# MiniMax-AI/VTP

Hardware: NVIDIA H100
Metric: images/sec (256x256 encode+decode+3-loss step) (higher is better)
Workload: dtype bf16

## Files before the change

vtp_b200/csrc/gemm.cu:

```cuda
#include <stdlib.h>

#include "host.h"
#include "ptx.cuh"

namespace vtp {

static constexpr int BM = 128;
static constexpr int BK = 64;
static constexpr int A_BYTES = BM * BK * 2;
static constexpr int NUM_THREADS = 512;
static constexpr int NUM_MMA_WARPS = 8;

struct GemmDev {
    int M, N, K;
    int a_mn, b_mn;
    int num_m_blocks, num_n_blocks, num_k_blocks, kb_per_split, num_splits;
    void* out;
    int ldo, out_dtype;
    const float* bias;
    int act, round_bf16;
    const void* resid;
    int ldr, resid_dtype;
    int accumulate;
    int rr_group, rr_skip;
    const __nv_bfloat16* rope_sin;
    const __nv_bfloat16* rope_cos;
    int rope_tokens, rope_prefix, rope_cols;
    int ps_r, ps_gh, ps_gw, ps_cout;
    __nv_bfloat16* out2;
    int ldo2;
    int conv_C, conv_H, conv_W, conv_TW, conv_TH, conv_tiles_h, conv_tiles_w, conv_B;
    const __nv_bfloat16* mask_pos;
    int ldm;
};

__device__ __forceinline__ float gelu_erf(float x) { return 0.5f * x * (1.0f + erff(x * 0.70710678118654752f)); }

static constexpr int STG_FLOATS = 32 * 32;
static constexpr int NUM_EPI_WARPS = 4;

__device__ __forceinline__ int stg_off(int r, int chunk ) { return r * 32 + ((chunk ^ (r & 7)) << 2); }

__device__ __forceinline__ long out_row(const GemmDev& p, int grow) {
    if (p.conv_C) {
// ... 246 lines not shown
            __syncwarp();
            store_bf16(p, stgb, lane, orow8, ocol0, 64, Nout, 0, has_resid);
            __syncwarp();
        }
        return;
    }
#pragma unroll
    for (int h = 0; h < 2; ++h) {
        if (32 * h < ncols) {
            stage_half(stg, lane, v, h);
            __syncwarp();
            store_half<PS>(p, stg, lane, grow0, orow8, ocol0, h, ncols, Nout, 0, has_resid);
            __syncwarp();
        }
    }
}


__device__ __forceinline__ int acc_key(int r) { return ((r & 3) << 1) | ((r >> 2) & 1); }

__device__ __forceinline__ void acc_ld32(const float* arow, int col0, int key, uint32_t (&r)[32]) {
#pragma unroll
    for (int i = 0; i < 8; ++i) {
        const float4 v = *reinterpret_cast<const float4*>(arow + col0 + 4 * (i ^ key));
        r[4 * i] = __float_as_uint(v.x), r[4 * i + 1] = __float_as_uint(v.y), r[4 * i + 2] = __float_as_uint(v.z),
        r[4 * i + 3] = __float_as_uint(v.w);
    }
}

struct AccHandoff {
    uint64_t* full;
    uint64_t* empty;
    uint32_t phase;
    __device__ __forceinline__ void wait_full() const { mbar_wait(full, phase); }
    __device__ __forceinline__ void release(int lane) const {
        __syncwarp();
        if (lane == 0) mbar_arrive(empty);
    }
};

struct TileIter {
    int n, m, ks;
    int dn, dm, dks;
    int nn, nm;
    __device__ __forceinline__ TileIter(int t0, int stride, int num_n, int num_m) : nn(num_n), nm(num_m) {
        n = t0 % num_n;
        const int r = t0 / num_n;
        m = r % num_m, ks = r / num_m;
        dn = stride % num_n;
        const int rs = stride / num_n;
        dm = rs % num_m, dks = rs / num_m;
    }
    __device__ __forceinline__ void next() {
        n += dn, m += dm, ks += dks;
        if (n >= nn) n -= nn, ++m;
        if (m >= nm) m -= nm, ++ks;
    }
};

template <int BN, int FAST>
__device__ __forceinline__ void fast_swiglu_tile(const GemmDev& p, const CUtensorMap* tmO, const CUtensorMap* tmO2, uint8_t* stg,
                                                 uint8_t* stg2, float* bias_s, int lane, int q, const AccHandoff& ah,
                                                 const float* arow, int key, int m_blk, int n0) {
    static_assert(BN == 128, "one packed chunk pair = one 64-column hidden line per tile row");
    constexpr bool PRE = FAST == 6;
    const int m0 = m_blk * BM;
    const int N = p.N;
// ... 153 lines not shown
                    if (ACT == VTP_ACT_RELU) {
#pragma unroll
                        for (int k = 0; k < 8; ++k) v[k] = fmaxf(v[k], 0.f);
                    }
                    uint4 w;
                    w.x = pack_bf16x2(v[0], v[1]), w.y = pack_bf16x2(v[2], v[3]);
                    w.z = pack_bf16x2(v[4], v[5]), w.w = pack_bf16x2(v[6], v[7]);
                    if (MASK) {
                        auto keep = [](uint32_t x, uint32_t mm) {
                            const uint32_t lo = ((mm & 0x7FFFu) != 0u && (mm & 0x8000u) == 0u) ? 0x0000FFFFu : 0u;
                            const uint32_t hi = ((mm & 0x7FFF0000u) != 0u && (mm & 0x80000000u) == 0u) ? 0xFFFF0000u : 0u;
                            return x & (lo | hi);
                        };
                        w.x = keep(w.x, rr[i].x), w.y = keep(w.y, rr[i].y), w.z = keep(w.z, rr[i].z), w.w = keep(w.w, rr[i].w);
                    } else if (RES) {
                        w.x = add_bf16x2(w.x, rr[i].x), w.y = add_bf16x2(w.y, rr[i].y), w.z = add_bf16x2(w.z, rr[i].z),
                        w.w = add_bf16x2(w.w, rr[i].w);
                    }
                    *reinterpret_cast<uint4*>(stg + stgb_off(lane, i)) = w;
                }
            }
            if (RES && !last) load_resid(col0 + CW);
            fence_proxy_async_smem();
            __syncwarp();
            if (lane == 0) {
                if (p.conv_C) tma_store_4d(tmO, stg, col0, ctx * p.conv_TW, cty * p.conv_TH + q * (32 / p.conv_TW), cb);
                else tma_store_2d(tmO, stg, col0, m0 + q * 32);
                bulk_commit();
            }
        }
    }
}

template <int BN, int STAGES, int TA, int TB>
__device__ __forceinline__ void gemm_mainloop(float (&acc)[BN / 2], uint8_t* ring, uint64_t* full_bar, uint64_t* empty_bar,
                                              int& s, uint32_t& ph, int nkb, int wg, int lane) {
    constexpr int STAGE_BYTES = A_BYTES + BN * BK * 2;
    int prev = -1;
    for (int kb = 0; kb < nkb; ++kb) {
        mbar_wait(&full_bar[s], ph);
        const uint32_t a_base = smem_u32(ring + s * STAGE_BYTES) + wg * 8192;
        const uint32_t b_base = smem_u32(ring + s * STAGE_BYTES + A_BYTES);
        wgmma_fence();
#pragma unroll
        for (int j = 0; j < BK / 16; ++j) {
            const uint64_t ad = TA ? wgmma_desc_sw128(a_base + j * 2048, 8192, 1024) : wgmma_desc_sw128(a_base + j * 32, 0, 1024);
            const uint64_t bd = TB ? wgmma_desc_sw128(b_base + j * 2048, 8192, 1024) : wgmma_desc_sw128(b_base + j * 32, 0, 1024);
            const uint32_t sc = (kb > 0 || j > 0) ? 1u : 0u;
            if constexpr (BN == 128) wgmma_m64n128_ss<TA, TB>(acc, ad, bd, sc);
            else wgmma_m64n64_ss<TA, TB>(acc, ad, bd, sc);
        }
        wgmma_commit();
        wgmma_wait<1>();
        fence_regs(acc);
        if (prev >= 0 && lane == 0) mbar_arrive(&empty_bar[prev]);
        prev = s;
        if (++s == STAGES) s = 0, ph ^= 1;
    }
    wgmma_wait<0>();
    fence_regs(acc);
    if (prev >= 0 && lane == 0) mbar_arrive(&empty_bar[prev]);
}

template <int BN, int STAGES, int ACT, bool PS, int FAST>
__global__ void __launch_bounds__(NUM_THREADS, 1)
gemm_kernel(const __grid_constant__ CUtensorMap tmA, const __grid_constant__ CUtensorMap tmB,
            const __grid_constant__ CUtensorMap tmO, const __grid_constant__ CUtensorMap tmO2, const GemmDev p) {
    static_assert(BN == 64 || BN == 128, "tile width");
    constexpr int B_BYTES = BN * BK * 2;
    constexpr int STAGE_BYTES = A_BYTES + B_BYTES;
    extern __shared__ __align__(1024) uint8_t smem_raw[];
    uint8_t* smem = reinterpret_cast<uint8_t*>((reinterpret_cast<uintptr_t>(smem_raw) + 1023) & ~uintptr_t(1023));
    constexpr int STG_BYTES = NUM_EPI_WARPS * STG_FLOATS * 4 * (FAST == 6 ? 2 : 1);
    uint8_t* ring = smem;
    float* acc_s = reinterpret_cast<float*>(ring + STAGES * STAGE_BYTES);
    float* stg_base = acc_s + BM * BN;
    float* bias_base = reinterpret_cast<float*>(reinterpret_cast<uint8_t*>(stg_base) + STG_BYTES);
    uint64_t* full_bar = reinterpret_cast<uint64_t*>(reinterpret_cast<uint8_t*>(bias_base) + (FAST ? NUM_EPI_WARPS * 256 : 0));
    uint64_t* empty_bar = full_bar + STAGES;
    uint64_t* acc_full = empty_bar + STAGES;
    uint64_t* acc_empty = acc_full + 1;

    const int warp = threadIdx.x >> 5;
    const int lane = threadIdx.x & 31;
    const int work_id = blockIdx.x;
    const int work_stride = gridDim.x;

    if (warp == 0 && lane == 0) {
        tma_prefetch_desc(&tmA);
        tma_prefetch_desc(&tmB);
        if (FAST) tma_prefetch_desc(&tmO);
        if (FAST == 6) tma_prefetch_desc(&tmO2);
        for (int s = 0; s < STAGES; ++s) mbar_init(&full_bar[s], 1), mbar_init(&empty_bar[s], NUM_MMA_WARPS);
        mbar_init(acc_full, NUM_MMA_WARPS);
        mbar_init(acc_empty, NUM_EPI_WARPS);
        fence_barrier_init();
    }
    __syncthreads();

    const int num_tiles = p.num_m_blocks * p.num_n_blocks * p.num_splits;
    if (warp < 4) {
        setmaxnreg_dec<40>();
        if (warp == 0 && lane == 0) {
            int s = 0;
            uint32_t ph = 0;
            TileIter ti(work_id, work_stride, p.num_n_blocks, p.num_m_blocks);
            for (int t = work_id; t < num_tiles; t += work_stride, ti.next()) {
                const int n_blk = ti.n, m_blk = ti.m, ks = ti.ks;
                const int kb0 = ks * p.kb_per_split;
                const int kb1 = min(kb0 + p.kb_per_split, p.num_k_blocks);
                const int m0 = m_blk * BM, n0 = n_blk * BN;
                int cv_x0 = 0, cv_y0 = 0, cv_b = 0, cv_c = 0, cv_dx = -1, cv_dy = -1;
                if (p.conv_C) {
                    cv_x0 = (m_blk % p.conv_tiles_w) * p.conv_TW;
                    cv_y0 = ((m_blk / p.conv_tiles_w) % p.conv_tiles_h) * p.conv_TH;
                    cv_b = m_blk / (p.conv_tiles_w * p.conv_tiles_h);
                    if (kb0 != 0) {
                        const int cpk = p.conv_C >> 6, tap = kb0 / cpk;
                        cv_c = (kb0 % cpk) << 6, cv_dx = tap % 3 - 1, cv_dy = tap / 3 - 1;
                    }
                }
                for (int kb = kb0; kb < kb1; ++kb) {
                    mbar_wait(&empty_bar[s], ph ^ 1);
                    uint8_t* sa = ring + s * STAGE_BYTES;
                    uint8_t* sb = sa + A_BYTES;
                    mbar_expect_tx(&full_bar[s], STAGE_BYTES);
                    const int k0 = kb * BK;
                    if (p.conv_C) {
                        tma_load_4d(sa, &tmA, &full_bar[s], cv_c, cv_x0 + cv_dx, cv_y0 + cv_dy, cv_b);
                        cv_c += 64;
                        if (cv_c == p.conv_C) {
                            cv_c = 0;
                            if (++cv_dx == 2) cv_dx = -1, ++cv_dy;
                        }
                    } else if (!p.a_mn) {
                        tma_load_2d(sa, &tmA, &full_bar[s], k0, m0);
                    } else {
                        tma_load_2d(sa, &tmA, &full_bar[s], m0, k0);
                        tma_load_2d(sa + 8192, &tmA, &full_bar[s], m0 + 64, k0);
                    }
                    if (!p.b_mn) {
                        tma_load_2d(sb, &tmB, &full_bar[s], k0, n0);
                    } else {
#pragma unroll
                        for (int i = 0; i < BN / 64; ++i) tma_load_2d(sb + i * 8192, &tmB, &full_bar[s], n0 + 64 * i, k0);
                    }
                    if (++s == STAGES) s = 0, ph ^= 1;
                }
            }
        }
    } else if (warp < 4 + NUM_MMA_WARPS) {
        setmaxnreg_inc<144>();
        const int wg = (warp >> 2) - 1;
        const int tw = threadIdx.x & 127;
        int s = 0;
        uint32_t ph = 0, acc_ph = 0;
        TileIter ti(work_id, work_stride, p.num_n_blocks, p.num_m_blocks);
        for (int t = work_id; t < num_tiles; t += work_stride, ti.next()) {
            const int kb0 = ti.ks * p.kb_per_split;
            const int nkb = min(kb0 + p.kb_per_split, p.num_k_blocks) - kb0;
            float acc[BN / 2];
            if (p.a_mn) {
                if (p.b_mn) gemm_mainloop<BN, STAGES, 1, 1>(acc, ring, full_bar, empty_bar, s, ph, nkb, wg, lane);
                else gemm_mainloop<BN, STAGES, 1, 0>(acc, ring, full_bar, empty_bar, s, ph, nkb, wg, lane);
            } else {
                if (p.b_mn) gemm_mainloop<BN, STAGES, 0, 1>(acc, ring, full_bar, empty_bar, s, ph, nkb, wg, lane);
                else gemm_mainloop<BN, STAGES, 0, 0>(acc, ring, full_bar, empty_bar, s, ph, nkb, wg, lane);
            }
            mbar_wait(acc_empty, acc_ph ^ 1);
            {
                const int r0 = 64 * wg + 16 * (tw >> 5) + ((tw & 31) >> 2), c0 = 2 * (tw & 3);
                const int key = acc_key(r0);
#pragma unroll
                for (int j = 0; j < BN / 8; ++j) {
                    const int off = 4 * ((2 * j + (c0 >> 2)) ^ key) + (c0 & 3);
                    *reinterpret_cast<float2*>(acc_s + r0 * BN + off) = make_float2(acc[4 * j], acc[4 * j + 1]);
                    *reinterpret_cast<float2*>(acc_s + (r0 + 8) * BN + off) = make_float2(acc[4 * j + 2], acc[4 * j + 3]);
                }
            }
            __syncwarp();
            if (lane == 0) mbar_arrive(acc_full);
            acc_ph ^= 1;
        }
    } else {
        setmaxnreg_inc<184>();
        const int q = warp & 3;
        float* stg = stg_base + q * STG_FLOATS;
        const bool has_resid = p.resid != nullptr;
        const float* arow = acc_s + (q * 32 + lane) * BN;
        const int key = acc_key(lane);
        AccHandoff ah{acc_full, acc_empty, 0};
        TileIter ti(work_id, work_stride, p.num_n_blocks, p.num_m_blocks);
        for (int t = work_id; t < num_tiles; t += work_stride, ti.next(), ah.phase ^= 1) {
            const int m_blk = ti.m, n0 = ti.n * BN;
            const int m0 = m_blk * BM;
            const int grow0 = m0 + q * 32;
            if constexpr (FAST == 6 || FAST == 7) {
                uint8_t* st1 = reinterpret_cast<uint8_t*>(stg);
                uint8_t* st2 = FAST == 6 ? reinterpret_cast<uint8_t*>(stg_base) + (NUM_EPI_WARPS + q) * STG_FLOATS * 4 : st1;
                fast_swiglu_tile<BN, FAST>(p, &tmO, &tmO2, st1, st2, bias_base + q * 64, lane, q, ah, arow, key, m_blk, n0);
                continue;
            }
            if constexpr (FAST != 0) {
                fast_epilogue_tile<BN, ACT, FAST>(p, &tmO, reinterpret_cast<uint8_t*>(stg), bias_base + q * 64, lane, q, ah,
                                                  arow, key, m_blk, n0);
                continue;
            }
            constexpr bool sw = ACT == VTP_ACT_SWIGLU8;
            long orow8[8];
#pragma unroll
            for (int it = 0; it < 8; ++it) orow8[it] = out_row(p, grow0 + 4 * it + (lane >> 3));
            uint32_t hold[16];
            ah.wait_full();
#pragma unroll 1
            for (int u = 0; u < BN / 64; ++u) {
                const int col0 = n0 + u * 64;
                if (col0 >= p.N) break;
                if (has_resid)
                    prefetch_resid_l2(p, lane, orow8, sw ? col0 >> 1 : col0, sw ? 32 : 64, sw ? p.N >> 1 : p.N);
                uint32_t r0[32], r1[32];
                acc_ld32(arow, u * 64, key, r0);
                acc_ld32(arow, u * 64 + 32, key, r1);
                if (u == BN / 64 - 1 || col0 + 64 >= p.N) ah.release(lane);
                float v[64];
#pragma unroll
                for (int i = 0; i < 32; ++i) v[i] = __uint_as_float(r0[i]), v[32 + i] = __uint_as_float(r1[i]);
                epilogue_unit<ACT, PS>(p, stg, lane, v, grow0, orow8, col0, has_resid, sw ? (u & 1) : 0, hold);
            }
        }
        if (FAST && lane == 0) bulk_wait0();
    }
}

template <int BN, int STAGES, int ACT, bool PS, int FAST = 0>
static int launch_gemm(const CUtensorMap& tmA, const CUtensorMap& tmB, const GemmDev& p, cudaStream_t stream,
                       const CUtensorMap* tmO = nullptr, const CUtensorMap* tmO2 = nullptr) {
    constexpr int smem_bytes = 1024 + STAGES * (A_BYTES + BN * BK * 2) + BM * BN * 4 +
                               NUM_EPI_WARPS * STG_FLOATS * 4 * (FAST == 6 ? 2 : 1) + (FAST ? NUM_EPI_WARPS * 256 : 0) +
                               (2 * STAGES + 2) * 8;
    static_assert(smem_bytes <= 232448, "shared memory budget (227 KB per block)");
    static bool configured = false;
    if (!configured) {
        VTP_CUDA(cudaFuncSetAttribute(gemm_kernel<BN, STAGES, ACT, PS, FAST>, cudaFuncAttributeMaxDynamicSharedMemorySize,
                                      smem_bytes));
        configured = true;
    }
    const int work = p.num_m_blocks * p.num_n_blocks * p.num_splits;
    const int grid = work < num_sms() ? work : num_sms();
    gemm_kernel<BN, STAGES, ACT, PS, FAST><<<grid, NUM_THREADS, smem_bytes, stream>>>(tmA, tmB, tmO ? *tmO : tmA,
                                                                                     tmO2 ? *tmO2 : tmA, p);
    VTP_LAUNCH_CHECK();
    return VTP_OK;
}

}

using namespace vtp;

extern "C" int vtp_gemm_bf16(const vtp_gemm_args* a, vtp_stream_t stream_) {
    cudaStream_t stream = reinterpret_cast<cudaStream_t>(stream_);
    VTP_CHECK_ARG(a != nullptr, "gemm: null args");
    VTP_CHECK_ARG(a->M > 0 && a->N > 0 && a->K > 0, "gemm: bad shape M=%d N=%d K=%d", a->M, a->N, a->K);
    VTP_CHECK_ARG(a->A && a->B && a->out, "gemm: null pointer");
    VTP_CHECK_ARG(a->lda % 8 == 0 && a->ldb % 8 == 0, "gemm: lda/ldb must be multiples of 8 (16B TMA strides)");
    VTP_CHECK_ARG((reinterpret_cast<uintptr_t>(a->A) & 15) == 0 && (reinterpret_cast<uintptr_t>(a->B) & 15) == 0,
                  "gemm: A/B must be 16B aligned");
    VTP_CHECK_ARG((reinterpret_cast<uintptr_t>(a->out) & 15) == 0, "gemm: out must be 16B aligned");
    VTP_CHECK_ARG(a->N % 8 == 0, "gemm: N must be a multiple of 8");
    VTP_CHECK_ARG(a->out_dtype == VTP_F32 || a->out_dtype == VTP_BF16, "gemm: bad out dtype");
    VTP_CHECK_ARG(a->ldo % (a->out_dtype == VTP_F32 ? 4 : 8) == 0 || a->ps_r > 0, "gemm: ldo alignment");
    int split_k = a->split_k < 1 ? 1 : a->split_k;
    const bool auto_split = a->split_k < 0 && a->accumulate && a->out_dtype == VTP_F32 && a->act == VTP_ACT_NONE && !a->bias;
    VTP_CHECK_ARG(split_k == 1 || (a->accumulate && a->out_dtype == VTP_F32 && a->act == VTP_ACT_NONE && !a->bias),
                  "gemm: split_k needs accumulate=1, fp32 out, no bias/activation");
    VTP_CHECK_ARG(!a->accumulate || a->out_dtype == VTP_F32, "gemm: accumulate needs fp32 out");
    if (a->act == VTP_ACT_ROPE)
        VTP_CHECK_ARG(a->rope_sin && a->rope_cos && a->rope_tokens > 0 && a->rope_cols % 64 == 0, "gemm: bad rope args");
    if (a->act == VTP_ACT_SWIGLU8) VTP_CHECK_ARG(a->N % 16 == 0, "gemm: swiglu needs N %% 16 == 0");
    if (a->ps_r > 0)
        VTP_CHECK_ARG(a->ps_r % 4 == 0 && a->M % (a->ps_gh * a->ps_gw) == 0 && a->N == a->ps_cout * a->ps_r * a->ps_r,
                      "gemm: bad pixel-shuffle args");
    if (a->resid) VTP_CHECK_ARG(a->ldr % (a->resid_dtype == VTP_F32 ? 4 : 8) == 0, "gemm: ldr alignment");
    if (a->out2) VTP_CHECK_ARG(a->ldo2 % 8 == 0, "gemm: ldo2 alignment");
// ... 23 lines not shown
        double best = -1.0;
        for (int sp = 1; sp <= 64 && sp * 8 <= (nkb > 8 ? nkb : 8); ++sp) {
            const int kps = ceil_div(nkb, sp);
            const int real = ceil_div(nkb, kps);
            const long work = (long)tiles * real;
            if (sp > 1 && work > 3L * grid) break;
            const double eff = (double)work / ((double)ceil_div((int)work, grid) * grid);
            if (eff > best + 0.02) best = eff, split_k = sp;
        }
    }

    GemmDev p;
    memset(&p, 0, sizeof(p));
    p.M = a->M, p.N = a->N, p.K = a->K;
    p.a_mn = a->a_mn_major ? 1 : 0, p.b_mn = a->b_mn_major ? 1 : 0;
    p.num_m_blocks = ceil_div(a->M, BM);
    p.num_n_blocks = ceil_div(a->N, BN);
    p.num_k_blocks = ceil_div(a->K, BK);
    p.kb_per_split = ceil_div(p.num_k_blocks, split_k);
    p.num_splits = ceil_div(p.num_k_blocks, p.kb_per_split);
    p.out = a->out, p.ldo = a->ldo, p.out_dtype = a->out_dtype;
    p.bias = a->bias, p.act = a->act, p.round_bf16 = a->round_bf16;
    p.resid = a->resid, p.ldr = a->ldr, p.resid_dtype = a->resid_dtype;
    p.accumulate = a->accumulate;
    p.rr_group = a->rr_group, p.rr_skip = a->rr_skip;
    p.rope_sin = reinterpret_cast<const __nv_bfloat16*>(a->rope_sin);
    p.rope_cos = reinterpret_cast<const __nv_bfloat16*>(a->rope_cos);
    p.rope_tokens = a->rope_tokens, p.rope_prefix = a->rope_prefix, p.rope_cols = a->rope_cols;
    p.ps_r = a->ps_r, p.ps_gh = a->ps_gh, p.ps_gw = a->ps_gw, p.ps_cout = a->ps_cout;
    p.out2 = reinterpret_cast<__nv_bfloat16*>(a->out2), p.ldo2 = a->ldo2;
    p.mask_pos = reinterpret_cast<const __nv_bfloat16*>(a->mask_pos), p.ldm = a->ldm;

    CUtensorMap tmA, tmB;
    if (conv) {
        const int W = a->conv_W, H = a->conv_H, Cc = a->conv_C, Bimg = a->M / (H * W);
        p.conv_C = Cc, p.conv_H = H, p.conv_W = W, p.conv_B = Bimg;
        p.conv_TW = (W % 16 == 0) ? 16 : (W % 8 == 0 ? 8 : 4);
        p.conv_TH = 128 / p.conv_TW;
        p.conv_tiles_w = W / p.conv_TW, p.conv_tiles_h = ceil_div(H, p.conv_TH);
        p.num_m_blocks = Bimg * p.conv_tiles_h * p.conv_tiles_w;
        p.M = p.num_m_blocks * 128;
        uint64_t dims[4] = {(uint64_t)Cc, (uint64_t)W, (uint64_t)H, (uint64_t)Bimg};
        uint64_t strides[3] = {(uint64_t)Cc * 2, (uint64_t)W * Cc * 2, (uint64_t)H * W * Cc * 2};
        uint32_t box[4] = {64, (uint32_t)p.conv_TW, (uint32_t)p.conv_TH, 1};
        int rc = make_tmap_bf16(&tmA, a->A, 4, dims, strides, box);
        if (rc) return rc;
    } else {
        uint64_t dims[2], strides[1] = {(uint64_t)a->lda * 2};
        uint32_t box[2];
        if (!p.a_mn) dims[0] = a->K, dims[1] = a->M, box[0] = 64, box[1] = 128;
        else dims[0] = a->M, dims[1] = a->K, box[0] = 64, box[1] = 64;
        int rc = make_tmap_bf16(&tmA, a->A, 2, dims, strides, box);
        if (rc) return rc;
    }
    {
        uint64_t dims[2], strides[1] = {(uint64_t)a->ldb * 2};
        uint32_t box[2];
        if (!p.b_mn) dims[0] = a->K, dims[1] = a->N, box[0] = 64, box[1] = (uint32_t)BN;
        else dims[0] = a->N, dims[1] = a->K, box[0] = 64, box[1] = 64;
        int rc = make_tmap_bf16(&tmB, a->B, 2, dims, strides, box);
        if (rc) return rc;
    }
    if (fast_swiglu) {
        CUtensorMap tmH, tmP;
        {
            uint64_t dims[2] = {(uint64_t)a->N / 2, (uint64_t)a->M}, strides[1] = {(uint64_t)a->ldo * 2};
            uint32_t box[2] = {64, 32};
            int rc = make_tmap(&tmH, a->out, VTP_BF16, 2, dims, strides, box);
            if (rc) return rc;
        }
        if (a->out2) {
            uint64_t dims[2] = {(uint64_t)a->N, (uint64_t)a->M}, strides[1] = {(uint64_t)a->ldo2 * 2};
            uint32_t box[2] = {64, 32};
            int rc = make_tmap(&tmP, a->out2, VTP_BF16, 2, dims, strides, box);
            if (rc) return rc;
            return launch_gemm<128, 4, VTP_ACT_SWIGLU8, false, 6>(tmA, tmB, p, stream, &tmH, &tmP);
        }
        return launch_gemm<128, 4, VTP_ACT_SWIGLU8, false, 7>(tmA, tmB, p, stream, &tmH);
    }
    if (fast) {
        CUtensorMap tmO;
        const int esz = a->out_dtype == VTP_F32 ? 4 : 2;
        int rc;
        if (conv) {
            uint64_t dims[4] = {(uint64_t)a->N, (uint64_t)p.conv_W, (uint64_t)p.conv_H, (uint64_t)p.conv_B};
            uint64_t strides[3] = {(uint64_t)a->ldo * 2, (uint64_t)p.conv_W * a->ldo * 2, (uint64_t)p.conv_H * p.conv_W * a->ldo * 2};
            uint32_t box[4] = {64, (uint32_t)p.conv_TW, (uint32_t)(32 / p.conv_TW), 1};
            rc = make_tmap(&tmO, a->out, VTP_BF16, 4, dims, strides, box);
        } else {
            uint64_t dims[2] = {(uint64_t)a->N, (uint64_t)a->M}, strides[1] = {(uint64_t)a->ldo * esz};
            uint32_t box[2] = {(uint32_t)(128 / esz), 32};
            rc = make_tmap(&tmO, a->out, a->out_dtype, 2, dims, strides, box);
        }
        if (rc) return rc;
        const int mode = a->mask_pos ? 5 : (a->out_dtype == VTP_F32 ? 3 : 1) + (a->resid ? 1 : 0);
#define VTP_FAST_CFG(ACT_, MODE_)                                                                                     \
    return BN == 64 ? launch_gemm<64, 4, ACT_, false, MODE_>(tmA, tmB, p, stream, &tmO)                              \
                    : launch_gemm<128, 4, ACT_, false, MODE_>(tmA, tmB, p, stream, &tmO)
        if (mode == 5) VTP_FAST_CFG(VTP_ACT_NONE, 5);
#define VTP_FAST_ACT(ACT_)                                 \
    do {                                                   \
        switch (mode) {                                    \
            case 1: VTP_FAST_CFG(ACT_, 1);                 \
            case 2: VTP_FAST_CFG(ACT_, 2);                 \
            case 3: VTP_FAST_CFG(ACT_, 3);                 \
            default: VTP_FAST_CFG(ACT_, 4);                \
        }                                                  \
    } while (0)
        if (a->act == VTP_ACT_RELU) VTP_FAST_ACT(VTP_ACT_RELU);
        VTP_FAST_ACT(VTP_ACT_NONE);
#undef VTP_FAST_ACT
#undef VTP_FAST_CFG
    }
#define VTP_LAUNCH(ACT_, PS_)                                                              \
    return BN == 64 ? launch_gemm<64, 4, ACT_, PS_>(tmA, tmB, p, stream)                  \
                    : launch_gemm<128, 4, ACT_, PS_>(tmA, tmB, p, stream)
    if (a->ps_r > 0) {
        VTP_CHECK_ARG(a->act == VTP_ACT_NONE, "gemm: pixel shuffle has no activation");
        VTP_LAUNCH(VTP_ACT_NONE, true);
    }
    switch (a->act) {
        case VTP_ACT_NONE: VTP_LAUNCH(VTP_ACT_NONE, false);
        case VTP_ACT_GELU: VTP_LAUNCH(VTP_ACT_GELU, false);
        case VTP_ACT_SWIGLU8: return launch_gemm<128, 4, VTP_ACT_SWIGLU8, false>(tmA, tmB, p, stream);
        case VTP_ACT_ROPE: VTP_LAUNCH(VTP_ACT_ROPE, false);
        case VTP_ACT_RELU: VTP_LAUNCH(VTP_ACT_RELU, false);
        default: VTP_FAIL(VTP_ERR_ARG, "gemm: unknown activation %d", a->act);
    }
#undef VTP_LAUNCH
}
```

vtp_b200/csrc/ptx.cuh:

```cuda
#pragma once
#include <cuda_runtime.h>
#include <cuda_bf16.h>
#include <cuda.h>
#include <stdint.h>

namespace vtp {

__device__ __forceinline__ uint32_t smem_u32(const void* p) {
    return static_cast<uint32_t>(__cvta_generic_to_shared(p));
}
__device__ __forceinline__ uint32_t lane_id() { return threadIdx.x & 31; }

__device__ __forceinline__ bool elect_one() {
    uint32_t pred;
    asm volatile(
        "{\n\t.reg .pred p;\n\t"
        "elect.sync _|p, 0xffffffff;\n\t"
        "selp.u32 %0, 1, 0, p;\n\t}\n"
        : "=r"(pred));
    return pred != 0;
}

__device__ __forceinline__ void mbar_init(uint64_t* bar, uint32_t count) {
    asm volatile("mbarrier.init.shared::cta.b64 [%0], %1;" ::"r"(smem_u32(bar)), "r"(count));
}
__device__ __forceinline__ void fence_barrier_init() {
    asm volatile("fence.mbarrier_init.release.cluster;" ::: "memory");
}
__device__ __forceinline__ void mbar_expect_tx(uint64_t* bar, uint32_t bytes) {
    asm volatile("mbarrier.arrive.expect_tx.shared::cta.b64 _, [%0], %1;" ::"r"(smem_u32(bar)), "r"(bytes)
                 : "memory");
}
__device__ __forceinline__ void mbar_arrive(uint64_t* bar) {
    asm volatile("mbarrier.arrive.shared::cta.b64 _, [%0];" ::"r"(smem_u32(bar)) : "memory");
}
__device__ __forceinline__ bool mbar_try_wait(uint64_t* bar, uint32_t parity) {
    uint32_t ok;
    asm volatile(
        "{\n\t.reg .pred p;\n\t"
        "mbarrier.try_wait.parity.shared::cta.b64 p, [%1], %2;\n\t"
        "selp.u32 %0, 1, 0, p;\n\t}\n"
        : "=r"(ok)
        : "r"(smem_u32(bar)), "r"(parity)
        : "memory");
    return ok != 0;
}
__device__ __forceinline__ void mbar_wait(uint64_t* bar, uint32_t parity) {
    while (!mbar_try_wait(bar, parity)) {
    }
}

__device__ __forceinline__ uint32_t cluster_ctarank() {
    uint32_t r;
    asm volatile("mov.u32 %0, %%cluster_ctarank;" : "=r"(r));
    return r;
}
__device__ __forceinline__ void cluster_sync() {
    asm volatile("barrier.cluster.arrive.release.aligned;\n\tbarrier.cluster.wait.acquire.aligned;" ::: "memory");
}
__device__ __forceinline__ uint32_t mapa_shared(uint32_t saddr, uint32_t rank) {
    uint32_t r;
    asm volatile("mapa.shared::cluster.u32 %0, %1, %2;" : "=r"(r) : "r"(saddr), "r"(rank));
    return r;
}
__device__ __forceinline__ float4 ld_shared_cluster_f4(uint32_t caddr) {
    float4 v;
    asm volatile("ld.shared::cluster.v4.f32 {%0, %1, %2, %3}, [%4];"
                 : "=f"(v.x), "=f"(v.y), "=f"(v.z), "=f"(v.w)
                 : "r"(caddr)
                 : "memory");
    return v;
}

__device__ __forceinline__ void fence_proxy_async_smem() {
    asm volatile("fence.proxy.async.shared::cta;" ::: "memory");
}

__device__ __forceinline__ void tma_prefetch_desc(const CUtensorMap* m) {
    asm volatile("prefetch.tensormap [%0];" ::"l"(reinterpret_cast<uint64_t>(m)) : "memory");
}
__device__ __forceinline__ void tma_load_2d(void* dst, const CUtensorMap* m, uint64_t* bar, int x, int y) {
    asm volatile(
// ... 133 lines not shown
```

Measured before the change: 700.5.

## Add ping-pong GEMM variant where two warpgroups alternate mainloop and epilogue

Adds a ping-pong kernel variant with 384 threads: one producer warpgroup plus two consumer warpgroups. Each consumer computes a full 128-row tile (two m64 wgmmas) and then runs that tile's epilogue itself, alternating tiles with the other consumer. Named barriers order mainloop turns and staging-buffer reuse. The goal is to overlap one tile's epilogue with the next tile's tensor-core work, replacing the separate epilogue warps. It is chosen when BN is 64 or there are at least 32 K-blocks per split. In exchange it needs 240 registers per consumer thread and adds more complex barrier phasing.

Result: no change. 703.2 (median of 6 runs) (+0.4%).

```diff
diff --git a/vtp_b200/csrc/gemm.cu b/vtp_b200/csrc/gemm.cu
--- a/vtp_b200/csrc/gemm.cu
+++ b/vtp_b200/csrc/gemm.cu
@@ -10,6 +10,7 @@
 static constexpr int A_BYTES = BM * BK * 2;
 static constexpr int NUM_THREADS = 512;
 static constexpr int NUM_MMA_WARPS = 8;
+static constexpr int PP_THREADS = 384;
 
 struct GemmDev {
     int M, N, K;
@@ -322,7 +323,16 @@
     uint64_t* full;
     uint64_t* empty;
     uint32_t phase;
-    __device__ __forceinline__ void wait_full() const { mbar_wait(full, phase); }
+    uint64_t* stg_free = nullptr;
+    int bar_id = 0;
+    __device__ __forceinline__ void wait_full() const {
+        if (bar_id) {
+            named_bar_sync(bar_id, 128);
+            mbar_wait(stg_free, phase);
+        } else {
+            mbar_wait(full, phase);
+        }
+    }
     __device__ __forceinline__ void release(int lane) const {
         __syncwarp();
         if (lane == 0) mbar_arrive(empty);
@@ -572,8 +582,50 @@
     if (prev >= 0 && lane == 0) mbar_arrive(&empty_bar[prev]);
 }
 
-template <int BN, int STAGES, int ACT, bool PS, int FAST>
-__global__ void __launch_bounds__(NUM_THREADS, 1)
+template <int BN, int STAGES, int TA, int TB>
+__device__ __forceinline__ void gemm_mainloop_pp(float (&acc0)[BN / 2], float (&acc1)[BN / 2], uint8_t* ring, uint64_t* full_bar,
+                                              uint64_t* empty_bar, int kpos, int nkb, int next_bar, int lane) {
+    constexpr int STAGE_BYTES = A_BYTES + BN * BK * 2;
+    int s = kpos % STAGES;
+    uint32_t ph = (kpos / STAGES) & 1;
+    int prev = -1;
+    for (int kb = 0; kb < nkb; ++kb) {
+        mbar_wait(&full_bar[s], ph);
+        const uint32_t a_base = smem_u32(ring + s * STAGE_BYTES);
+        const uint32_t b_base = smem_u32(ring + s * STAGE_BYTES + A_BYTES);
+        wgmma_fence();
+#pragma unroll
+        for (int j = 0; j < BK / 16; ++j) {
+            const uint64_t ad0 = TA ? wgmma_desc_sw128(a_base + j * 2048, 8192, 1024) : wgmma_desc_sw128(a_base + j * 32, 0, 1024);
+            const uint64_t ad1 = TA ? wgmma_desc_sw128(a_base + 8192 + j * 2048, 8192, 1024)
+                                    : wgmma_desc_sw128(a_base + 8192 + j * 32, 0, 1024);
+            const uint64_t bd = TB ? wgmma_desc_sw128(b_base + j * 2048, 8192, 1024) : wgmma_desc_sw128(b_base + j * 32, 0, 1024);
+            const uint32_t sc = (kb > 0 || j > 0) ? 1u : 0u;
+            if constexpr (BN == 128) {
+                wgmma_m64n128_ss<TA, TB>(acc0, ad0, bd, sc);
+                wgmma_m64n128_ss<TA, TB>(acc1, ad1, bd, sc);
+            } else {
+                wgmma_m64n64_ss<TA, TB>(acc0, ad0, bd, sc);
+                wgmma_m64n64_ss<TA, TB>(acc1, ad1, bd, sc);
+            }
+        }
+        wgmma_commit();
+        if (kb == nkb - 1 && next_bar) named_bar_arrive(next_bar, 256);
+        wgmma_wait<1>();
+        fence_regs(acc0);
+        fence_regs(acc1);
+        if (prev >= 0 && lane == 0) mbar_arrive(&empty_bar[prev]);
+        prev = s;
+        if (++s == STAGES) s = 0, ph ^= 1;
+    }
+    wgmma_wait<0>();
+    fence_regs(acc0);
+    fence_regs(acc1);
+    if (prev >= 0 && lane == 0) mbar_arrive(&empty_bar[prev]);
+}
+
+template <int BN, int STAGES, int ACT, bool PS, int FAST, bool PP>
+__global__ void __launch_bounds__(PP ? PP_THREADS : NUM_THREADS, 1)
 gemm_kernel(const __grid_constant__ CUtensorMap tmA, const __grid_constant__ CUtensorMap tmB,
             const __grid_constant__ CUtensorMap tmO, const __grid_constant__ CUtensorMap tmO2, const GemmDev p) {
     static_assert(BN == 64 || BN == 128, "tile width");
@@ -601,8 +653,8 @@
         tma_prefetch_desc(&tmB);
         if (FAST) tma_prefetch_desc(&tmO);
         if (FAST == 6) tma_prefetch_desc(&tmO2);
-        for (int s = 0; s < STAGES; ++s) mbar_init(&full_bar[s], 1), mbar_init(&empty_bar[s], NUM_MMA_WARPS);
-        mbar_init(acc_full, NUM_MMA_WARPS);
+        for (int s = 0; s < STAGES; ++s) mbar_init(&full_bar[s], 1), mbar_init(&empty_bar[s], PP ? 4 : NUM_MMA_WARPS);
+        mbar_init(acc_full, PP ? 4 : NUM_MMA_WARPS);
         mbar_init(acc_empty, NUM_EPI_WARPS);
         fence_barrier_init();
     }
@@ -610,7 +662,8 @@
 
     const int num_tiles = p.num_m_blocks * p.num_n_blocks * p.num_splits;
     if (warp < 4) {
-        setmaxnreg_dec<40>();
+        if constexpr (PP) setmaxnreg_dec<24>();
+        else setmaxnreg_dec<40>();
         if (warp == 0 && lane == 0) {
             int s = 0;
             uint32_t ph = 0;
@@ -659,6 +712,92 @@
                 }
             }
         }
+    } else if constexpr (PP) {
+        uint64_t* const acc_free = acc_empty;
+        uint64_t* const stg_free = acc_full;
+        setmaxnreg_inc<240>();
+        const int wg = __shfl_sync(0xffffffffu, (warp >> 2) - 1, 0);
+        const int tw = threadIdx.x & 127;
+        const int q = warp & 3;
+        float* stg = stg_base + q * STG_FLOATS;
+        const bool has_resid = p.resid != nullptr;
+        const float* arow = acc_s + (q * 32 + lane) * BN;
+        const int key = acc_key(lane);
+        const AccHandoff ah{acc_full , acc_free, (uint32_t)(wg ^ 1), stg_free, 3 + wg};
+        const int my_turn = 1 + wg, other_turn = 2 - wg;
+        int kpos = 0;
+        TileIter ti(work_id, work_stride, p.num_n_blocks, p.num_m_blocks);
+        for (int t = work_id, j = 0; t < num_tiles; t += work_stride, ti.next(), ++j) {
+            const int kb0 = ti.ks * p.kb_per_split;
+            const int nkb = min(kb0 + p.kb_per_split, p.num_k_blocks) - kb0;
+            if ((j & 1) != wg) {
+                kpos += nkb;
+                continue;
+            }
+            const int next_bar = t + work_stride < num_tiles ? other_turn : 0;
+            if (j > 0) named_bar_sync(my_turn, 256);
+            float acc0[BN / 2], acc1[BN / 2];
+#pragma unroll
+            for (int i = 0; i < BN / 2; ++i) acc0[i] = 0.f, acc1[i] = 0.f;
+            if (p.a_mn) {
+                if (p.b_mn) gemm_mainloop_pp<BN, STAGES, 1, 1>(acc0, acc1, ring, full_bar, empty_bar, kpos, nkb, next_bar, lane);
+                else gemm_mainloop_pp<BN, STAGES, 1, 0>(acc0, acc1, ring, full_bar, empty_bar, kpos, nkb, next_bar, lane);
+            } else {
+                if (p.b_mn) gemm_mainloop_pp<BN, STAGES, 0, 1>(acc0, acc1, ring, full_bar, empty_bar, kpos, nkb, next_bar, lane);
+                else gemm_mainloop_pp<BN, STAGES, 0, 0>(acc0, acc1, ring, full_bar, empty_bar, kpos, nkb, next_bar, lane);
+            }
+            kpos += nkb;
+            mbar_wait(acc_free, ah.phase);
+            {
+                const int r0 = 16 * (tw >> 5) + ((tw & 31) >> 2), c0 = 2 * (tw & 3);
+                const int key0 = acc_key(r0);
+#pragma unroll
+                for (int jj = 0; jj < BN / 8; ++jj) {
+                    const int off = 4 * ((2 * jj + (c0 >> 2)) ^ key0) + (c0 & 3);
+                    *reinterpret_cast<float2*>(acc_s + r0 * BN + off) = make_float2(acc0[4 * jj], acc0[4 * jj + 1]);
+                    *reinterpret_cast<float2*>(acc_s + (r0 + 8) * BN + off) = make_float2(acc0[4 * jj + 2], acc0[4 * jj + 3]);
+                    *reinterpret_cast<float2*>(acc_s + (r0 + 64) * BN + off) = make_float2(acc1[4 * jj], acc1[4 * jj + 1]);
+                    *reinterpret_cast<float2*>(acc_s + (r0 + 72) * BN + off) = make_float2(acc1[4 * jj + 2], acc1[4 * jj + 3]);
+                }
+            }
+            const int m_blk = ti.m, n0 = ti.n * BN;
+            const int m0 = m_blk * BM;
+            const int grow0 = m0 + q * 32;
+            if constexpr (FAST == 6 || FAST == 7) {
+                uint8_t* st1 = reinterpret_cast<uint8_t*>(stg);
+                uint8_t* st2 = FAST == 6 ? reinterpret_cast<uint8_t*>(stg_base) + (NUM_EPI_WARPS + q) * STG_FLOATS * 4 : st1;
+                fast_swiglu_tile<BN, FAST>(p, &tmO, &tmO2, st1, st2, bias_base + q * 64, lane, q, ah, arow, key, m_blk, n0);
+            } else if constexpr (FAST != 0) {
+                fast_epilogue_tile<BN, ACT, FAST>(p, &tmO, reinterpret_cast<uint8_t*>(stg), bias_base + q * 64, lane, q, ah,
+                                                  arow, key, m_blk, n0);
+            } else {
+                constexpr bool sw = ACT == VTP_ACT_SWIGLU8;
+                long orow8[8];
+#pragma unroll
+                for (int it = 0; it < 8; ++it) orow8[it] = out_row(p, grow0 + 4 * it + (lane >> 3));
+                uint32_t hold[16];
+                ah.wait_full();
+#pragma unroll 1
+                for (int u = 0; u < BN / 64; ++u) {
+                    const int col0 = n0 + u * 64;
+                    if (col0 >= p.N) break;
+                    if (has_resid)
+                        prefetch_resid_l2(p, lane, orow8, sw ? col0 >> 1 : col0, sw ? 32 : 64, sw ? p.N >> 1 : p.N);
+                    uint32_t r0[32], r1[32];
+                    acc_ld32(arow, u * 64, key, r0);
+                    acc_ld32(arow, u * 64 + 32, key, r1);
+                    if (u == BN / 64 - 1 || col0 + 64 >= p.N) ah.release(lane);
+                    float v[64];
+#pragma unroll
+                    for (int i = 0; i < 32; ++i) v[i] = __uint_as_float(r0[i]), v[32 + i] = __uint_as_float(r1[i]);
+                    epilogue_unit<ACT, PS>(p, stg, lane, v, grow0, orow8, col0, has_resid, sw ? (u & 1) : 0, hold);
+                }
+            }
+            if (FAST && lane == 0) bulk_wait_read0();
+            __syncwarp();
+            if (lane == 0) mbar_arrive(stg_free);
+        }
+        if (FAST && lane == 0) bulk_wait0();
     } else if (warp < 4 + NUM_MMA_WARPS) {
         setmaxnreg_inc<144>();
         const int wg = (warp >> 2) - 1;
@@ -749,16 +888,21 @@
                                NUM_EPI_WARPS * STG_FLOATS * 4 * (FAST == 6 ? 2 : 1) + (FAST ? NUM_EPI_WARPS * 256 : 0) +
                                (2 * STAGES + 2) * 8;
     static_assert(smem_bytes <= 232448, "shared memory budget (227 KB per block)");
-    static bool configured = false;
-    if (!configured) {
-        VTP_CUDA(cudaFuncSetAttribute(gemm_kernel<BN, STAGES, ACT, PS, FAST>, cudaFuncAttributeMaxDynamicSharedMemorySize,
-                                      smem_bytes));
-        configured = true;
+    const bool pp = BN == 64 || p.kb_per_split >= 32;
+    static bool configured[2] = {false, false};
+    if (!configured[pp]) {
+        if (pp) VTP_CUDA(cudaFuncSetAttribute(gemm_kernel<BN, STAGES, ACT, PS, FAST, true>,
+                                              cudaFuncAttributeMaxDynamicSharedMemorySize, smem_bytes));
+        else VTP_CUDA(cudaFuncSetAttribute(gemm_kernel<BN, STAGES, ACT, PS, FAST, false>,
+                                           cudaFuncAttributeMaxDynamicSharedMemorySize, smem_bytes));
+        configured[pp] = true;
     }
     const int work = p.num_m_blocks * p.num_n_blocks * p.num_splits;
     const int grid = work < num_sms() ? work : num_sms();
-    gemm_kernel<BN, STAGES, ACT, PS, FAST><<<grid, NUM_THREADS, smem_bytes, stream>>>(tmA, tmB, tmO ? *tmO : tmA,
-                                                                                     tmO2 ? *tmO2 : tmA, p);
+    const CUtensorMap& o1 = tmO ? *tmO : tmA;
+    const CUtensorMap& o2 = tmO2 ? *tmO2 : tmA;
+    if (pp) gemm_kernel<BN, STAGES, ACT, PS, FAST, true><<<grid, PP_THREADS, smem_bytes, stream>>>(tmA, tmB, o1, o2, p);
+    else gemm_kernel<BN, STAGES, ACT, PS, FAST, false><<<grid, NUM_THREADS, smem_bytes, stream>>>(tmA, tmB, o1, o2, p);
     VTP_LAUNCH_CHECK();
     return VTP_OK;
 }
diff --git a/vtp_b200/csrc/ptx.cuh b/vtp_b200/csrc/ptx.cuh
--- a/vtp_b200/csrc/ptx.cuh
+++ b/vtp_b200/csrc/ptx.cuh
@@ -48,6 +48,13 @@
 __device__ __forceinline__ void mbar_wait(uint64_t* bar, uint32_t parity) {
     while (!mbar_try_wait(bar, parity)) {
     }
+}
+
+__device__ __forceinline__ void named_bar_sync(int id, int count) {
+    asm volatile("bar.sync %0, %1;" ::"r"(id), "r"(count) : "memory");
+}
+__device__ __forceinline__ void named_bar_arrive(int id, int count) {
+    asm volatile("bar.arrive %0, %1;" ::"r"(id), "r"(count) : "memory");
 }
 
 __device__ __forceinline__ uint32_t cluster_ctarank() {
```

## Load conv halo slabs once and reuse across three vertical taps

Applied to the files above, without the earlier changes.

For implicit-GEMM 3x3 convolutions, the producer now loads one taller A slab (tile height plus two halo rows) per channel block and x-offset. The MMA warps then reuse it for the three dy taps by offsetting the smem descriptor by a row of the tile, instead of issuing a separate A TMA load per tap. A second barrier ring manages slab lifetimes. The K iteration order changes to dy-innermost, which reindexes the B weight loads. Freed smem allows more B stages (8 or 5), and the path is restricted to split_k=1, non-transposed B, and none/relu activations. The aim is to cut A-side TMA traffic roughly threefold, at the cost of extra barrier logic and a dependency on the weight layout's tap ordering.

Result: no change. 703.8 before, 709.6 after (median of 6 runs) (+0.8%).

```diff
diff --git a/vtp_b200/csrc/gemm.cu b/vtp_b200/csrc/gemm.cu
--- a/vtp_b200/csrc/gemm.cu
+++ b/vtp_b200/csrc/gemm.cu
@@ -542,15 +542,31 @@
     }
 }
 
-template <int BN, int STAGES, int TA, int TB>
+__host__ __device__ constexpr int halo_slabs(int stages) { return 1 + (stages + 2) / 3; }
+static constexpr int HALO_STAGES_64 = 8, HALO_STAGES_128 = 5;
+static constexpr int HALO_SLAB_BYTES = (BM + 2 * 16) * BK * 2;
+
+struct HaloRing {
+    uint8_t* slabs;
+    uint64_t* full;
+    uint64_t* empty;
+    int sl;
+    uint32_t ph;
+};
+
+template <int BN, int STAGES, int TA, int TB, bool HALO>
 __device__ __forceinline__ void gemm_mainloop(float (&acc)[BN / 2], uint8_t* ring, uint64_t* full_bar, uint64_t* empty_bar,
-                                              int& s, uint32_t& ph, int nkb, int wg, int lane) {
-    constexpr int STAGE_BYTES = A_BYTES + BN * BK * 2;
+                                              int& s, uint32_t& ph, int nkb, int wg, int lane, HaloRing& hr, int tw_bytes) {
+    constexpr int A_STAGE = HALO ? 0 : A_BYTES;
+    constexpr int STAGE_BYTES = A_STAGE + BN * BK * 2;
     int prev = -1;
+    int dy = 0, prev_dy = 0, prev_sl = 0;
     for (int kb = 0; kb < nkb; ++kb) {
+        if (HALO && dy == 0) mbar_wait(&hr.full[hr.sl], hr.ph);
         mbar_wait(&full_bar[s], ph);
-        const uint32_t a_base = smem_u32(ring + s * STAGE_BYTES) + wg * 8192;
-        const uint32_t b_base = smem_u32(ring + s * STAGE_BYTES + A_BYTES);
+        const uint32_t a_base = HALO ? smem_u32(hr.slabs + hr.sl * HALO_SLAB_BYTES) + wg * 8192 + dy * tw_bytes
+                                     : smem_u32(ring + s * STAGE_BYTES) + wg * 8192;
+        const uint32_t b_base = smem_u32(ring + s * STAGE_BYTES + A_STAGE);
         wgmma_fence();
 #pragma unroll
         for (int j = 0; j < BK / 16; ++j) {
@@ -563,33 +579,51 @@
         wgmma_commit();
         wgmma_wait<1>();
         fence_regs(acc);
-        if (prev >= 0 && lane == 0) mbar_arrive(&empty_bar[prev]);
+        if (prev >= 0 && lane == 0) {
+            mbar_arrive(&empty_bar[prev]);
+            if (HALO && prev_dy == 2) mbar_arrive(&hr.empty[prev_sl]);
+        }
         prev = s;
         if (++s == STAGES) s = 0, ph ^= 1;
+        if constexpr (HALO) {
+            prev_dy = dy, prev_sl = hr.sl;
+            if (++dy == 3) {
+                dy = 0;
+                if (++hr.sl == halo_slabs(STAGES)) hr.sl = 0, hr.ph ^= 1;
+            }
+        }
     }
     wgmma_wait<0>();
     fence_regs(acc);
-    if (prev >= 0 && lane == 0) mbar_arrive(&empty_bar[prev]);
-}
-
-template <int BN, int STAGES, int ACT, bool PS, int FAST>
+    if (prev >= 0 && lane == 0) {
+        mbar_arrive(&empty_bar[prev]);
+        if (HALO && prev_dy == 2) mbar_arrive(&hr.empty[prev_sl]);
+    }
+}
+
+template <int BN, int STAGES, int ACT, bool PS, int FAST, bool HALO>
 __global__ void __launch_bounds__(NUM_THREADS, 1)
 gemm_kernel(const __grid_constant__ CUtensorMap tmA, const __grid_constant__ CUtensorMap tmB,
             const __grid_constant__ CUtensorMap tmO, const __grid_constant__ CUtensorMap tmO2, const GemmDev p) {
     static_assert(BN == 64 || BN == 128, "tile width");
     constexpr int B_BYTES = BN * BK * 2;
-    constexpr int STAGE_BYTES = A_BYTES + B_BYTES;
+    constexpr int STAGE_BYTES = (HALO ? 0 : A_BYTES) + B_BYTES;
+    constexpr int SLABS = halo_slabs(STAGES);
+    constexpr int SLAB_RING_BYTES = HALO ? SLABS * HALO_SLAB_BYTES : 0;
     extern __shared__ __align__(1024) uint8_t smem_raw[];
     uint8_t* smem = reinterpret_cast<uint8_t*>((reinterpret_cast<uintptr_t>(smem_raw) + 1023) & ~uintptr_t(1023));
     constexpr int STG_BYTES = NUM_EPI_WARPS * STG_FLOATS * 4 * (FAST == 6 ? 2 : 1);
     uint8_t* ring = smem;
-    float* acc_s = reinterpret_cast<float*>(ring + STAGES * STAGE_BYTES);
+    uint8_t* slabs = ring + STAGES * STAGE_BYTES;
+    float* acc_s = reinterpret_cast<float*>(slabs + SLAB_RING_BYTES);
     float* stg_base = acc_s + BM * BN;
     float* bias_base = reinterpret_cast<float*>(reinterpret_cast<uint8_t*>(stg_base) + STG_BYTES);
     uint64_t* full_bar = reinterpret_cast<uint64_t*>(reinterpret_cast<uint8_t*>(bias_base) + (FAST ? NUM_EPI_WARPS * 256 : 0));
     uint64_t* empty_bar = full_bar + STAGES;
     uint64_t* acc_full = empty_bar + STAGES;
     uint64_t* acc_empty = acc_full + 1;
+    uint64_t* slab_full = acc_empty + 1;
+    uint64_t* slab_empty = slab_full + SLABS;
 
     const int warp = threadIdx.x >> 5;
     const int lane = threadIdx.x & 31;
@@ -604,6 +638,8 @@
         for (int s = 0; s < STAGES; ++s) mbar_init(&full_bar[s], 1), mbar_init(&empty_bar[s], NUM_MMA_WARPS);
         mbar_init(acc_full, NUM_MMA_WARPS);
         mbar_init(acc_empty, NUM_EPI_WARPS);
+        if (HALO)
+            for (int s = 0; s < SLABS; ++s) mbar_init(&slab_full[s], 1), mbar_init(&slab_empty[s], NUM_MMA_WARPS);
         fence_barrier_init();
     }
     __syncthreads();
@@ -612,8 +648,8 @@
     if (warp < 4) {
         setmaxnreg_dec<40>();
         if (warp == 0 && lane == 0) {
-            int s = 0;
-            uint32_t ph = 0;
+            int s = 0, hsl = 0;
+            uint32_t ph = 0, hph = 0;
             TileIter ti(work_id, work_stride, p.num_n_blocks, p.num_m_blocks);
             for (int t = work_id; t < num_tiles; t += work_stride, ti.next()) {
                 const int n_blk = ti.n, m_blk = ti.m, ks = ti.ks;
@@ -630,32 +666,53 @@
                         cv_c = (kb0 % cpk) << 6, cv_dx = tap % 3 - 1, cv_dy = tap / 3 - 1;
                     }
                 }
-                for (int kb = kb0; kb < kb1; ++kb) {
-                    mbar_wait(&empty_bar[s], ph ^ 1);
-                    uint8_t* sa = ring + s * STAGE_BYTES;
-                    uint8_t* sb = sa + A_BYTES;
-                    mbar_expect_tx(&full_bar[s], STAGE_BYTES);
-                    const int k0 = kb * BK;
-                    if (p.conv_C) {
-                        tma_load_4d(sa, &tmA, &full_bar[s], cv_c, cv_x0 + cv_dx, cv_y0 + cv_dy, cv_b);
-                        cv_c += 64;
-                        if (cv_c == p.conv_C) {
-                            cv_c = 0;
-                            if (++cv_dx == 2) cv_dx = -1, ++cv_dy;
+                if constexpr (HALO) {
+                    const uint32_t slab_bytes = (p.conv_TH + 2) * p.conv_TW * BK * 2;
+                    for (int kb = kb0; kb < kb1; ++kb) {
+                        if (cv_dy == -1) {
+                            mbar_wait(&slab_empty[hsl], hph ^ 1);
+                            mbar_expect_tx(&slab_full[hsl], slab_bytes);
+                            tma_load_4d(slabs + hsl * HALO_SLAB_BYTES, &tmA, &slab_full[hsl], cv_c, cv_x0 + cv_dx, cv_y0 - 1, cv_b);
                         }
-                    } else if (!p.a_mn) {
-                        tma_load_2d(sa, &tmA, &full_bar[s], k0, m0);
-                    } else {
-                        tma_load_2d(sa, &tmA, &full_bar[s], m0, k0);
-                        tma_load_2d(sa + 8192, &tmA, &full_bar[s], m0 + 64, k0);
+                        mbar_wait(&empty_bar[s], ph ^ 1);
+                        uint8_t* sb = ring + s * STAGE_BYTES;
+                        mbar_expect_tx(&full_bar[s], B_BYTES);
+                        tma_load_2d(sb, &tmB, &full_bar[s], ((cv_dy + 1) * 3 + cv_dx + 1) * p.conv_C + cv_c, n0);
+                        if (++s == STAGES) s = 0, ph ^= 1;
+                        if (++cv_dy == 2) {
+                            cv_dy = -1;
+                            if (++hsl == SLABS) hsl = 0, hph ^= 1;
+                            if (++cv_dx == 2) cv_dx = -1, cv_c += 64;
+                        }
                     }
-                    if (!p.b_mn) {
-                        tma_load_2d(sb, &tmB, &full_bar[s], k0, n0);
-                    } else {
-#pragma unroll
-                        for (int i = 0; i < BN / 64; ++i) tma_load_2d(sb + i * 8192, &tmB, &full_bar[s], n0 + 64 * i, k0);
+                } else {
+                    for (int kb = kb0; kb < kb1; ++kb) {
+                        mbar_wait(&empty_bar[s], ph ^ 1);
+                        uint8_t* sa = ring + s * STAGE_BYTES;
+                        uint8_t* sb = sa + A_BYTES;
+                        mbar_expect_tx(&full_bar[s], STAGE_BYTES);
+                        const int k0 = kb * BK;
+                        if (p.conv_C) {
+                            tma_load_4d(sa, &tmA, &full_bar[s], cv_c, cv_x0 + cv_dx, cv_y0 + cv_dy, cv_b);
+                            cv_c += 64;
+                            if (cv_c == p.conv_C) {
+                                cv_c = 0;
+                                if (++cv_dx == 2) cv_dx = -1, ++cv_dy;
+                            }
+                        } else if (!p.a_mn) {
+                            tma_load_2d(sa, &tmA, &full_bar[s], k0, m0);
+                        } else {
+                            tma_load_2d(sa, &tmA, &full_bar[s], m0, k0);
+                            tma_load_2d(sa + 8192, &tmA, &full_bar[s], m0 + 64, k0);
+                        }
+                        if (!p.b_mn) {
+                            tma_load_2d(sb, &tmB, &full_bar[s], k0, n0);
+                        } else {
+#pragma unroll
+                            for (int i = 0; i < BN / 64; ++i) tma_load_2d(sb + i * 8192, &tmB, &full_bar[s], n0 + 64 * i, k0);
+                        }
+                        if (++s == STAGES) s = 0, ph ^= 1;
                     }
-                    if (++s == STAGES) s = 0, ph ^= 1;
                 }
             }
         }
@@ -665,17 +722,21 @@
         const int tw = threadIdx.x & 127;
         int s = 0;
         uint32_t ph = 0, acc_ph = 0;
+        HaloRing hr{slabs, slab_full, slab_empty, 0, 0};
+        const int tw_bytes = p.conv_TW * BK * 2;
         TileIter ti(work_id, work_stride, p.num_n_blocks, p.num_m_blocks);
         for (int t = work_id; t < num_tiles; t += work_stride, ti.next()) {
             const int kb0 = ti.ks * p.kb_per_split;
             const int nkb = min(kb0 + p.kb_per_split, p.num_k_blocks) - kb0;
             float acc[BN / 2];
-            if (p.a_mn) {
-                if (p.b_mn) gemm_mainloop<BN, STAGES, 1, 1>(acc, ring, full_bar, empty_bar, s, ph, nkb, wg, lane);
-                else gemm_mainloop<BN, STAGES, 1, 0>(acc, ring, full_bar, empty_bar, s, ph, nkb, wg, lane);
+            if constexpr (HALO) {
+                gemm_mainloop<BN, STAGES, 0, 0, true>(acc, ring, full_bar, empty_bar, s, ph, nkb, wg, lane, hr, tw_bytes);
+            } else if (p.a_mn) {
+                if (p.b_mn) gemm_mainloop<BN, STAGES, 1, 1, false>(acc, ring, full_bar, empty_bar, s, ph, nkb, wg, lane, hr, 0);
+                else gemm_mainloop<BN, STAGES, 1, 0, false>(acc, ring, full_bar, empty_bar, s, ph, nkb, wg, lane, hr, 0);
             } else {
-                if (p.b_mn) gemm_mainloop<BN, STAGES, 0, 1>(acc, ring, full_bar, empty_bar, s, ph, nkb, wg, lane);
-                else gemm_mainloop<BN, STAGES, 0, 0>(acc, ring, full_bar, empty_bar, s, ph, nkb, wg, lane);
+                if (p.b_mn) gemm_mainloop<BN, STAGES, 0, 1, false>(acc, ring, full_bar, empty_bar, s, ph, nkb, wg, lane, hr, 0);
+                else gemm_mainloop<BN, STAGES, 0, 0, false>(acc, ring, full_bar, empty_bar, s, ph, nkb, wg, lane, hr, 0);
             }
             mbar_wait(acc_empty, acc_ph ^ 1);
             {
@@ -742,23 +803,24 @@
     }
 }
 
-template <int BN, int STAGES, int ACT, bool PS, int FAST = 0>
+template <int BN, int STAGES, int ACT, bool PS, int FAST = 0, bool HALO = false>
 static int launch_gemm(const CUtensorMap& tmA, const CUtensorMap& tmB, const GemmDev& p, cudaStream_t stream,
                        const CUtensorMap* tmO = nullptr, const CUtensorMap* tmO2 = nullptr) {
-    constexpr int smem_bytes = 1024 + STAGES * (A_BYTES + BN * BK * 2) + BM * BN * 4 +
+    constexpr int smem_bytes = 1024 + STAGES * ((HALO ? 0 : A_BYTES) + BN * BK * 2) +
+                               (HALO ? halo_slabs(STAGES) * HALO_SLAB_BYTES : 0) + BM * BN * 4 +
                                NUM_EPI_WARPS * STG_FLOATS * 4 * (FAST == 6 ? 2 : 1) + (FAST ? NUM_EPI_WARPS * 256 : 0) +
-                               (2 * STAGES + 2) * 8;
+                               (2 * STAGES + 2 + 2 * halo_slabs(STAGES)) * 8;
     static_assert(smem_bytes <= 232448, "shared memory budget (227 KB per block)");
     static bool configured = false;
     if (!configured) {
-        VTP_CUDA(cudaFuncSetAttribute(gemm_kernel<BN, STAGES, ACT, PS, FAST>, cudaFuncAttributeMaxDynamicSharedMemorySize,
+        VTP_CUDA(cudaFuncSetAttribute(gemm_kernel<BN, STAGES, ACT, PS, FAST, HALO>, cudaFuncAttributeMaxDynamicSharedMemorySize,
                                       smem_bytes));
         configured = true;
     }
     const int work = p.num_m_blocks * p.num_n_blocks * p.num_splits;
     const int grid = work < num_sms() ? work : num_sms();
-    gemm_kernel<BN, STAGES, ACT, PS, FAST><<<grid, NUM_THREADS, smem_bytes, stream>>>(tmA, tmB, tmO ? *tmO : tmA,
-                                                                                     tmO2 ? *tmO2 : tmA, p);
+    gemm_kernel<BN, STAGES, ACT, PS, FAST, HALO><<<grid, NUM_THREADS, smem_bytes, stream>>>(tmA, tmB, tmO ? *tmO : tmA,
+                                                                                           tmO2 ? *tmO2 : tmA, p);
     VTP_LAUNCH_CHECK();
     return VTP_OK;
 }
@@ -848,6 +910,7 @@
     p.mask_pos = reinterpret_cast<const __nv_bfloat16*>(a->mask_pos), p.ldm = a->ldm;
 
     CUtensorMap tmA, tmB;
+    bool halo = false;
     if (conv) {
         const int W = a->conv_W, H = a->conv_H, Cc = a->conv_C, Bimg = a->M / (H * W);
         p.conv_C = Cc, p.conv_H = H, p.conv_W = W, p.conv_B = Bimg;
@@ -856,9 +919,11 @@
         p.conv_tiles_w = W / p.conv_TW, p.conv_tiles_h = ceil_div(H, p.conv_TH);
         p.num_m_blocks = Bimg * p.conv_tiles_h * p.conv_tiles_w;
         p.M = p.num_m_blocks * 128;
+        halo = p.conv_TW >= 8 && split_k == 1 && !p.b_mn && (a->act == VTP_ACT_NONE || a->act == VTP_ACT_RELU) &&
+               (BN == 64 || (Cc >= 256 && H >= 32)) && getenv("VTP_GEMM_CONV_NO_HALO") == nullptr;
         uint64_t dims[4] = {(uint64_t)Cc, (uint64_t)W, (uint64_t)H, (uint64_t)Bimg};
         uint64_t strides[3] = {(uint64_t)Cc * 2, (uint64_t)W * Cc * 2, (uint64_t)H * W * Cc * 2};
-        uint32_t box[4] = {64, (uint32_t)p.conv_TW, (uint32_t)p.conv_TH, 1};
+        uint32_t box[4] = {64, (uint32_t)p.conv_TW, (uint32_t)(p.conv_TH + (halo ? 2 : 0)), 1};
         int rc = make_tmap_bf16(&tmA, a->A, 4, dims, strides, box);
         if (rc) return rc;
     } else {
@@ -913,6 +978,15 @@
 #define VTP_FAST_CFG(ACT_, MODE_)                                                                                     \
     return BN == 64 ? launch_gemm<64, 4, ACT_, false, MODE_>(tmA, tmB, p, stream, &tmO)                              \
                     : launch_gemm<128, 4, ACT_, false, MODE_>(tmA, tmB, p, stream, &tmO)
+#define VTP_HALO_CFG(ACT_, MODE_)                                                                                     \
+    return BN == 64 ? launch_gemm<64, HALO_STAGES_64, ACT_, false, MODE_, true>(tmA, tmB, p, stream, &tmO)           \
+                    : launch_gemm<128, HALO_STAGES_128, ACT_, false, MODE_, true>(tmA, tmB, p, stream, &tmO)
+        if (halo) {
+            if (mode == 5) VTP_HALO_CFG(VTP_ACT_NONE, 5);
+            if (a->act == VTP_ACT_RELU) VTP_HALO_CFG(VTP_ACT_RELU, 1);
+            VTP_HALO_CFG(VTP_ACT_NONE, 1);
+        }
+#undef VTP_HALO_CFG
         if (mode == 5) VTP_FAST_CFG(VTP_ACT_NONE, 5);
 #define VTP_FAST_ACT(ACT_)                                 \
     do {                                                   \
@@ -931,6 +1005,13 @@
 #define VTP_LAUNCH(ACT_, PS_)                                                              \
     return BN == 64 ? launch_gemm<64, 4, ACT_, PS_>(tmA, tmB, p, stream)                  \
                     : launch_gemm<128, 4, ACT_, PS_>(tmA, tmB, p, stream)
+    if (halo) {
+        if (a->act == VTP_ACT_RELU)
+            return BN == 64 ? launch_gemm<64, HALO_STAGES_64, VTP_ACT_RELU, false, 0, true>(tmA, tmB, p, stream)
+                            : launch_gemm<128, HALO_STAGES_128, VTP_ACT_RELU, false, 0, true>(tmA, tmB, p, stream);
+        return BN == 64 ? launch_gemm<64, HALO_STAGES_64, VTP_ACT_NONE, false, 0, true>(tmA, tmB, p, stream)
+                        : launch_gemm<128, HALO_STAGES_128, VTP_ACT_NONE, false, 0, true>(tmA, tmB, p, stream);
+    }
     if (a->ps_r > 0) {
         VTP_CHECK_ARG(a->act == VTP_ACT_NONE, "gemm: pixel shuffle has no activation");
         VTP_LAUNCH(VTP_ACT_NONE, true);
```
